# ColumbiaDVMM/ColumbiaImageSearch

Measured on AMD Instinct MI355X. Metric: queries/sec @ recall@10 on 10M LOPQ index, higher is better.
Workload: dtype f64

## Files before the change

### columbiaimagesearch_amd/csrc/lopq_scan3.hip

```cpp
#include "scan_common.h"
#include <cmath>
#include <cstdio>
#include <cstdlib>

typedef unsigned short u16x2_t __attribute__((ext_vector_type(2)));

static __device__ __forceinline__ uint32_t pk_add_u16(uint32_t a, uint32_t b) {
    return __builtin_bit_cast(uint32_t, (u16x2_t)(__builtin_bit_cast(u16x2_t, a) + __builtin_bit_cast(u16x2_t, b)));
}
static __device__ __forceinline__ uint32_t pk_subsat_u16(uint32_t a, uint32_t b) {
    return __builtin_bit_cast(uint32_t, __builtin_elementwise_sub_sat(__builtin_bit_cast(u16x2_t, a), __builtin_bit_cast(u16x2_t, b)));
}

static __device__ __forceinline__ uint32_t pk_min_u16(uint32_t a, uint32_t b) {
    return __builtin_bit_cast(uint32_t, __builtin_elementwise_min(__builtin_bit_cast(u16x2_t, a), __builtin_bit_cast(u16x2_t, b)));
}

static const int S3G = 4;

#ifdef CIS_S3_COUNTERS
__device__ unsigned long long g_s3_ctr[16];
#define S3_CLK() ((long long)__builtin_amdgcn_s_memtime())
#define S3_CTR(i, v) do { if (threadIdx.x == 0) atomicAdd(&g_s3_ctr[i], (unsigned long long)(v)); } while (0)
extern "C" int cis_debug_counters3(unsigned long long* out, int reset) {
// ... 60 lines not shown
        if (boundW < lds_ld(&sh->wt[w])) lds_st(&sh->wt[w], boundW);
    }
    __builtin_amdgcn_fence(__ATOMIC_RELEASE, "workgroup");
    uint32_t thr = bound_to_thr(block_bound<NW>(sh), qs.inv_up);
    uint32_t cut = thr;
    int W = cap - L;
    W = W > 24 ? 24 : (W < 0 ? 0 : W);
    if (wave_count_le<NR>(keep, s, cut) > L + W) {
        const uint32_t v = wave_bisect_window<NR>(keep, s, mn, mx, L, W);
        const uint32_t vm = v + (uint32_t)M;
        if (wave_count_le<NR>(keep, s, vm) > cap) return -1;
        const uint64_t boundL = val_to_bound(v, M, qs.ub);
        if (lane == 0) {
            if (boundL < lds_ld(&sh->wl[w])) lds_st(&sh->wl[w], boundL);
        }
        __builtin_amdgcn_fence(__ATOMIC_RELEASE, "workgroup");
        thr = bound_to_thr(block_bound<NW>(sh), qs.inv_up);
        cut = vm < thr ? vm : thr;
    }
    if (lane == 0) {
        if (thr < lds_ld(&sh->thr)) lds_st(&sh->thr, thr);
    }
    return wave_stable_keep<NR>([&](int r) { return keep[r] && s[r] <= cut; }, [&](int r, int idx) { rk[idx] = ent[r]; });
}

template <int M, int NR, int NW>
__device__ __forceinline__ int wave_compact3_exact(uint32_t* rk, int cnt, int L, int Lw, const QScale& qs, Scan3Shared* sh, int w,
                                                   const uint8_t* __restrict__ codes, int64_t start, int K,
                                                   const double* __restrict__ t0, const double* __restrict__ t1, uint32_t& dup_pos) {
    const int lane = threadIdx.x & 63;
    uint32_t hi[NR], lo[NR], ent[NR];
    bool keep[NR];
    uint32_t mn = 0xffffffffu, mx = 0u;
#pragma unroll
    for (int r = 0; r < NR; ++r) {
        const int e = r * 64 + lane;
        keep[r] = e < cnt;
        ent[r] = keep[r] ? rk[e] : 0xffffffffu;
        hi[r] = 0xffffffffu;
        lo[r] = 0xffffffffu;
    }
#pragma unroll
    for (int r = 0; r < NR; ++r) {
        if (r * 64 >= cnt) break;
        const CodeWords<M> cw = load_code<M>(codes, start + (keep[r] ? (ent[r] & 0xffffu) : 0u));
        const uint64_t k = keep[r] ? (uint64_t)__double_as_longlong(adc64_words<M>(cw.w, K, t0, t1)) : ~0ull;
        hi[r] = (uint32_t)(k >> 32);
        lo[r] = (uint32_t)k;
        mn = (keep[r] && hi[r] < mn) ? hi[r] : mn;
        mx = (keep[r] && hi[r] > mx) ? hi[r] : mx;
    }
    wave_minmax_all(mn, mx);
    uint32_t vhiL;
    uint64_t boundL;
    wave_exact_cut<NR>(hi, lo, keep, [&](int r) { return ent[r] & 0xffffu; }, mn, mx, cnt, L, vhiL, boundL, dup_pos);
    const uint64_t boundW = (cnt >= Lw) ? hi_to_bound(wave_kth_bisect<NR>(hi, keep, mn, vhiL, Lw)) : 0x7ff0000000000000ull;
    if (lane == 0) {
        if (boundW < lds_ld(&sh->wt[w])) lds_st(&sh->wt[w], boundW);
        if (boundL < lds_ld(&sh->wl[w])) lds_st(&sh->wl[w], boundL);
    }
    __builtin_amdgcn_fence(__ATOMIC_RELEASE, "workgroup");
    const uint64_t bound = block_bound<NW>(sh);
    if (lane == 0) {
        const uint32_t thr = bound_to_thr(bound, qs.inv_up);
        if (thr < lds_ld(&sh->thr)) lds_st(&sh->thr, thr);
    }
    return wave_stable_keep<NR>([&](int r) { return keep[r] && (((uint64_t)hi[r] << 32) | lo[r]) <= bound; },
                                [&](int r, int idx) { rk[idx] = ent[r]; });
}

template <int NR, int NW>
__device__ __forceinline__ int wave_filter3(uint32_t* rk, int cnt, const QScale& qs, const Scan3Shared* sh) {
    const int lane = threadIdx.x & 63;
    const uint32_t thr = bound_to_thr(block_bound<NW>(sh), qs.inv_up);
    uint32_t k[NR];
#pragma unroll
    for (int r = 0; r < NR; ++r) {
        const int e = r * 64 + lane;
        k[r] = e < cnt ? rk[e] : 0xffffffffu;
    }
    return wave_stable_keep<NR>([&](int r) { return (r * 64 + lane < cnt) && ((k[r] >> 16) <= thr); }, [&](int r, int idx) { rk[idx] = k[r]; });
}

template <int M, int OCT>
__device__ __forceinline__ void adc16_issue(const uint32_t (&D)[(M + 3) / 4], int o, const char* __restrict__ tab,
                                            const RotConsts<M>& rc, u32x2_t (&f)[OCT]) {
    constexpr int SH = ((M == 4) ? 2 : (M == 8 ? 3 : 4)) + 3;
#pragma unroll
    for (int i = 0; i < OCT; ++i) {
        const int t = o * OCT + i;
        const uint32_t k = __builtin_amdgcn_ubfe(D[t >> 2], rc.sh[t & 3], 8);
        f[i] = *reinterpret_cast<const u32x2_t*>(tab + ((k << SH) | (rc.cj[t] << 1)));
    }
}

template <int OCT>
__device__ __forceinline__ u32x2_t adc16_sum(const u32x2_t (&f)[OCT]) {
    uint32_t a0 = f[0][0], a1 = f[0][1];
#pragma unroll
    for (int i = 1; i < OCT; ++i) {
        a0 = pk_add_u16(a0, f[i][0]);
        a1 = pk_add_u16(a1, f[i][1]);
    }
    u32x2_t r;
    r[0] = a0; r[1] = a1;
    return r;
}

static __device__ __forceinline__ uint32_t ld16(const uint16_t* p) { return *reinterpret_cast<const volatile uint16_t*>(p); }
static __device__ __forceinline__ void st16(uint16_t* p, uint32_t v) { *reinterpret_cast<volatile uint16_t*>(p) = (uint16_t)v; }

template <int M, int NR, int U, int NW>
__device__ __forceinline__ void scan3_group(const WorkItem* __restrict__ items, const TabDesc* __restrict__ tabs,
                                            const int (&item_idx)[S3G], int ng,
                                            const double* __restrict__ T, const float* __restrict__ T32,
                                            const uint8_t* __restrict__ codes, int K, int L, int S,
                                            uint64_t* __restrict__ item_surv, int* __restrict__ item_n, float* __restrict__ item_slack,
                                            unsigned long long* __restrict__ qbound, char* smem, bool two_pass) {
    constexpr int G = S3G;
    constexpr int R = NR * 64 - 8;
    constexpr int nf = M / 2;
    constexpr int OCT = M >= 8 ? 8 : 4, NU = M / OCT;
    constexpr uint32_t CAP = 65535u / M;
    char* tab = smem;
    uint32_t* rk_all = reinterpret_cast<uint32_t*>(smem + (size_t)K * M * G * 2);
    Scan3Shared* sh = reinterpret_cast<Scan3Shared*>(rk_all + G * NW * R);
    uint16_t* thr1 = reinterpret_cast<uint16_t*>(sh + G);
    const int tid = threadIdx.x, lane = tid & 63;
    const int w = __builtin_amdgcn_readfirstlane(tid >> 6);
    const long long c0 = S3_CLK();
    (void)c0;
    const WorkItem it0 = items[item_idx[0]];
    {
        int tab0[G], tab1[G];
        float qinv[G];
#pragma unroll
        for (int g = 0; g < G; ++g) {
            tab0[g] = items[item_idx[g]].tab0; tab1[g] = items[item_idx[g]].tab1;
            float mxT = fmaxf(__int_as_float(tabs[tab0[g]].pad), __int_as_float(tabs[tab1[g]].pad));
            mxT = fmaxf(mxT, 1e-30f);
            float qi = ((float)CAP / mxT) * (1.0f - 9.5367431640625e-7f);
            qi = (mxT < 3.0e38f) ? qi : 0.0f;
            qi = (qi < 3.0e38f) ? qi : 3.0e38f;
            qinv[g] = qi;
        }
        if (tid < G) {
            const int g = tid;
            float qi = qinv[0];
#pragma unroll
            for (int gg = 1; gg < G; ++gg) qi = (g == gg) ? qinv[gg] : qi;
            const double inv_up = (double)qi * (1.0 + 2.384185791015625e-7);
            const double ub = qi > 0.0f ? (1.0 + 4.76837158203125e-7) / (double)qi : __longlong_as_double(0x7ff0000000000000LL);
            sh[g].inv_up = inv_up;
            sh[g].ub = ub;
            const unsigned long long e = (g < ng) ? __hip_atomic_load(&qbound[items[item_idx[g]].q], __ATOMIC_RELAXED, __HIP_MEMORY_SCOPE_AGENT)
                                                  : 0x7ff0000000000000ull;
            sh[g].ext = e;
            uint32_t thr = (g < ng) ? bound_to_thr(e, inv_up) : 0u;
#ifdef CIS_S3_PROBE_NOPASS
            thr = 0u;
            if (true) { sh[g].thr = 0u; thr1[g] = 0; } else
#endif
            { sh[g].thr = thr; thr1[g] = (uint16_t)((g < ng) ? thr + 1u : 0u); }
            if (g < ng) {
                item_slack[2 * (int64_t)item_idx[g] + 0] = __double2float_ru(ub * ((double)M + 0.1));
                item_slack[2 * (int64_t)item_idx[g] + 1] = __double2float_ru(ub);
            }
        }
        if (tid < 8 * G) {
            const int g = tid >> 3, i = tid & 7;
            sh[g].wt[i] = 0x7ff0000000000000ull; sh[g].wl[i] = 0x7ff0000000000000ull;
            sh[g].wcnt[i] = 0;
        }
        const int nvec = (nf * K) >> 2;
        uint32_t* tw = reinterpret_cast<uint32_t*>(tab);
// ... 460 lines not shown
    const uint8_t* __restrict__ codes, int K, int L, int S, int* __restrict__ queue_ctr ,
    uint64_t* __restrict__ item_surv, int* __restrict__ item_n, float* __restrict__ item_slack,
    unsigned long long* __restrict__ qbound , int two_pass, int single_queue ) {
    extern __shared__ __attribute__((aligned(16))) char smem[];
    constexpr int G = S3G;
    constexpr int R = NR * 64 - 8;
    int* s_next = reinterpret_cast<int*>(smem + (size_t)K * M * G * 2 + (size_t)G * NW * R * 4 + G * sizeof(Scan3Shared) + 32);
    const int* qs = n_slots_ptr + 8;
    const int home = blockIdx.x & 7;
    const long long k0 = S3_CLK();
    (void)k0;
    for (int a = 0; a < 8; ++a) {
        const int x = (home + a) & 7;
        const int qstart = qs[x];
        const int count = single_queue ? (x == 0 ? qs[1] - qstart : 0) : qs[x + 1] - qstart;
        if (count <= 0) continue;
        while (true) {
            const long long q0 = S3_CLK();
            (void)q0;
            int j;
            if constexpr (NW > 1) {
                __syncthreads();
                if (threadIdx.x == 0) *s_next = atomicAdd(&queue_ctr[x], 1);
                __syncthreads();
                j = __builtin_amdgcn_readfirstlane(*s_next);
            } else {
                int t = 0;
                if (threadIdx.x == 0) t = atomicAdd(&queue_ctr[x], 1);
                j = __builtin_amdgcn_readfirstlane(t);
            }
            S3_CTR(8, S3_CLK() - q0);
            if (j >= count) break;
            const int slot = qstart + j;
            int idx[G];
            int ng = 0;
            bool same = true;
#pragma unroll
            for (int g = 0; g < G; ++g) {
                idx[g] = slots[slot * G + g];
                if (idx[g] >= 0) {
                    ng = g + 1;
                    same = same && items[idx[g]].start == items[idx[0]].start && items[idx[g]].len == items[idx[0]].len;
                } else {
                    idx[g] = idx[0];
                }
            }
            if (!same) {
                for (int g2 = 0; g2 < ng; ++g2) {
                    int oi[G];
#pragma unroll
                    for (int g = 0; g < G; ++g) {
                        oi[g] = idx[0];
#pragma unroll
                        for (int gg = 1; gg < G; ++gg)
                            if (gg == g2) oi[g] = idx[gg];
                    }
                    if (g2 > 0) __syncthreads();
                    scan3_group<M, NR, U, NW>(items, tabs, oi, 1, T, T32, codes, K, L, S, item_surv, item_n, item_slack, qbound, smem, two_pass != 0);
                }
                continue;
            }
            scan3_group<M, NR, U, NW>(items, tabs, idx, ng, T, T32, codes, K, L, S, item_surv, item_n, item_slack, qbound, smem, two_pass != 0);
        }
    }
    S3_CTR(9, S3_CLK() - k0);
    S3_CTR(10, 1);
}

struct Slot4 {
    int item[S3G], tab0[S3G], tab1[S3G], q[S3G];
    float qinv[S3G];
    int start_lo, start_hi, len, ng;
    int ist_lo[S3G], ist_hi[S3G], ilen[S3G];
};
struct Scan4Shared {
    double inv_up, ub;
    uint64_t ext;
    uint32_t tau;
    int verify;
    int cnt;
    int q;
};

template <int M, int UU, int OCT = (M >= 8 ? 8 : 4)>
__device__ __forceinline__ void adc16_rows(const CodeWords<M> (&cur)[UU], const char* __restrict__ tab, const RotConsts<M>& rc,
                                           u32x2_t (&d)[UU]) {
    constexpr int NU = M / OCT;
    u32x2_t fbuf[2][OCT];
    uint32_t D[2][(M + 3) / 4];
    rot_words<M>(cur[0], rc, D[0]);
    adc16_issue<M, OCT>(D[0], 0, tab, rc, fbuf[0]);
#pragma unroll
    for (int q = 0; q < UU * NU; ++q) {
        const int u = q / NU, o = q % NU;
        if (q + 1 < UU * NU) {
            const int u1 = (q + 1) / NU, o1 = (q + 1) % NU;
            if (o1 == 0) rot_words<M>(cur[u1], rc, D[u1 & 1]);
            adc16_issue<M, OCT>(D[u1 & 1], o1, tab, rc, fbuf[(q + 1) & 1]);
        }
        __builtin_amdgcn_sched_barrier(0);
        const u32x2_t part = adc16_sum<OCT>(fbuf[q & 1]);
        if (o == 0) {
            d[u] = part;
        } else {
            d[u][0] = pk_add_u16(d[u][0], part[0]);
            d[u][1] = pk_add_u16(d[u][1], part[1]);
        }
        __builtin_amdgcn_sched_barrier(0);
    }
}

static __device__ __forceinline__ void lds_barrier() {
    asm volatile("s_waitcnt lgkmcnt(0)\n\ts_barrier" ::: "memory");
}

#ifndef CIS_S4_U
#define CIS_S4_U 2
#endif
#ifndef CIS_S4_UL
#define CIS_S4_UL 2
#endif
#ifndef CIS_S4_OCT
#define CIS_S4_OCT 4
#endif
#ifndef CIS_S4_WPE
#define CIS_S4_WPE 6
#endif
static const int S4_OCT = CIS_S4_OCT;
#ifndef CIS_S4_DEFER
#define CIS_S4_DEFER 1
#endif
#ifndef CIS_S4_NW_LONG
#define CIS_S4_NW_LONG 4
#endif
#ifndef CIS_S4_NW_SHORT
#define CIS_S4_NW_SHORT 4
#endif
#ifndef CIS_S4_WPE8
#define CIS_S4_WPE8 6
#endif
#ifndef CIS_S4_GLISTS
#define CIS_S4_GLISTS 0
#endif
#ifndef CIS_S4_WPE_LONG
#define CIS_S4_WPE_LONG 6
#endif
#ifndef CIS_S4_PF
#define CIS_S4_PF 2
#endif
#ifndef CIS_S4_LCAP
#define CIS_S4_LCAP 504
#endif
#ifndef CIS_S4_NS
#define CIS_S4_NS 16
#endif
#ifndef CIS_S4_Z
#define CIS_S4_Z 4.0f
#endif
static const int S4_DS = 8;
static const int S4_LCAP = CIS_S4_LCAP;
static const int S4_NS = CIS_S4_NS;

static const int S4_LCAP_LONG = 1016;

static size_t scan4_lds(int M, int K, int lcap, int nw) {
    const bool glists = lcap > 504 && CIS_S4_DEFER != 0 && CIS_S4_GLISTS != 0;
    const size_t lists = glists ? (size_t)nw * ((32 / nw) * 128) * 2 : (size_t)S3G * lcap * 4, samp = glists ? 0 : (size_t)S3G * S4_NS * 64 * 2;
    return (size_t)K * M * S3G * 2 + (lists > samp ? lists : samp) + S3G * sizeof(Scan4Shared) + 32 + (size_t)S3G * nw * 4 + (S4_DS + 1) * sizeof(Slot4);
}

static __device__ __forceinline__ int sample_row(int t, int nrows, int ns) { return (int)(((uint32_t)t * (uint32_t)nrows) / (uint32_t)ns); }

template <int M, int U, int NW, int WPE, int LCAPT>
__global__ __launch_bounds__(NW * 64) __attribute__((amdgpu_waves_per_eu(WPE, WPE))) void k_adc_scan4(
    const WorkItem* __restrict__ items, const TabDesc* __restrict__ tabs, const int* __restrict__ slots,
    const int* __restrict__ n_slots_ptr, const float* __restrict__ T32 , const double* __restrict__ T,
    const uint8_t* __restrict__ codes, int K, int L, int S,
    int* __restrict__ dbg , int* __restrict__ fhdr ,
    int* __restrict__ fslots, uint64_t* __restrict__ item_surv, int* __restrict__ item_n, float* __restrict__ item_slack,
    unsigned long long* __restrict__ qbound, float zq , int frac_den ,
    int nsx , int dyn ,
    float sat ) {
    extern __shared__ __attribute__((aligned(16))) char smem[];
    constexpr int G = S3G;
    static_assert(NW >= G && NW % G == 0 && NW <= 8, "waves 0 .. G-1 serve one query each in the threshold and verification phases");
    static_assert(M == 4 || M == 8 || M == 16, "float4s of the half tables are dealt to the threads in rounds of 256");
    constexpr int nf = M / 2;
    constexpr uint32_t CAP = 65535u / M;
    constexpr int LCAP = LCAPT, NS = S4_NS, NRV = (LCAP + 63) / 64;
    constexpr bool GLISTS = (LCAPT > 504) && (CIS_S4_DEFER != 0) && (CIS_S4_GLISTS != 0);
    constexpr size_t LIST_B_FULL = (size_t)G * LCAP * 4 > (size_t)G * NS * 64 * 2 ? (size_t)G * LCAP * 4 : (size_t)G * NS * 64 * 2;
    constexpr size_t LIST_B = GLISTS ? (size_t)NW * (((LCAPT > 504 ? 32 : 16) / NW) * 128) * 2 : LIST_B_FULL;
    char* tab = smem;
    uint32_t* lists = reinterpret_cast<uint32_t*>(smem + (size_t)K * M * G * 2);
    uint16_t* samp = reinterpret_cast<uint16_t*>(lists);
    Scan4Shared* sh = reinterpret_cast<Scan4Shared*>(reinterpret_cast<char*>(lists) + LIST_B);
    uint16_t* thr1 = reinterpret_cast<uint16_t*>(sh + G);
    int* s_flag = reinterpret_cast<int*>(thr1 + 4);
    int* s_cnt = s_flag + 1;
    int* wcnt = reinterpret_cast<int*>(reinterpret_cast<char*>(thr1) + 32);
    Slot4* sd = reinterpret_cast<Slot4*>(reinterpret_cast<char*>(thr1) + 32 + G * NW * 4);
#ifdef CIS_S4_SHARED_LISTS
    constexpr bool WLISTS = LCAPT > 504;
#else
    constexpr bool WLISTS = true;
#endif
    constexpr int WCAP = LCAPT / NW;
    constexpr int PCAP_LDS = (int)(LIST_B / (NW * 2));
    constexpr int NRP = (LCAPT > 504 ? 32 : 16) / NW;
    constexpr int PCAP = NRP * 128 < PCAP_LDS ? NRP * 128 : PCAP_LDS;
    static_assert(PCAP % 2 == 0 && (PCAP_LDS * 2) % 4 == 0, "position lists are read back as 32-bit pairs");
    const int tid = threadIdx.x, lane = tid & 63;
    const int w = __builtin_amdgcn_readfirstlane(tid >> 6);
    const int total = n_slots_ptr[0];
    const int xcd = blockIdx.x & 7, lb = blockIdx.x >> 3;
    const int LW = gridDim.x >> 3;
    auto slot_of = [&](int k) -> int {
        const int li = lb + k * LW;
        const int j = (((li >> 5) * 8 + xcd) << 5) | (li & 31);
        return j < total ? j : -1;
    };
    const RotConsts<M> rc = make_rot<M>(lane);
    const int nvec = (nf * K) >> 2;
    const long long k0 = S3_CLK();
    (void)k0;
    for (int kb = 0;; kb += S4_DS) {
        int dyn_j = -1;
        if (LCAPT > 504 && dyn) {
            __syncthreads();
            if (tid == 0) {
                int jn = -1;
                if (dyn == 1) {
                    jn = atomicAdd(&dbg[6], 1);
                    jn = jn < total ? jn : -1;
                } else {
                    int* qx = dbg - 9;
                    for (int a2 = 0; a2 < 8 && jn < 0; ++a2) {
                        const int x = (xcd + a2) & 7;
                        const int li = atomicAdd(&qx[x], 1);
                        const int jj = (((li >> 5) * 8 + x) << 5) | (li & 31);
                        if (jj < total) jn = jj;
                    }
                }
                *s_flag = jn;
            }
            __syncthreads();
            dyn_j = *s_flag;
            if (dyn_j < 0) break;
        } else {
            if (slot_of(kb) < 0) break;
        }
        __syncthreads();
        if (tid < S4_DS) {
            Slot4 d;
            int dyn_s = dyn;
            asm volatile("" : "+s"(dyn_s));
            const int j = (LCAPT > 504 && dyn_s) ? (tid == 0 ? dyn_j : -1) : slot_of(kb + tid);
            d.ng = 0; d.len = 0; d.start_lo = d.start_hi = 0;
#pragma unroll
            for (int g = 0; g < G; ++g) { d.item[g] = 0; d.tab0[g] = 0; d.tab1[g] = 0; d.q[g] = 0; d.qinv[g] = 0.f; d.ist_lo[g] = d.ist_hi[g] = d.ilen[g] = 0; }
            if (j >= 0) {
                int idx[G];
                int ng = 0;
                bool same = true;
#pragma unroll
                for (int g = 0; g < G; ++g) idx[g] = slots[j * G + g];
                const int64_t st0 = items[idx[0]].start;
                const int len0 = items[idx[0]].len;
#pragma unroll
                for (int g = 0; g < G; ++g) {
                    if (idx[g] >= 0) ng = g + 1;
                    else idx[g] = idx[0];
                    const WorkItem* it = &items[idx[g]];
                    same = same && it->start == st0 && it->len == len0;
                    const int t0 = it->tab0, t1 = it->tab1;
                    d.item[g] = idx[g]; d.tab0[g] = t0; d.tab1[g] = t1; d.q[g] = it->q;
                    d.ist_lo[g] = (int)(uint32_t)it->start; d.ist_hi[g] = (int)(it->start >> 32); d.ilen[g] = it->len;
                    float mxT = fmaxf(__int_as_float(tabs[t0].pad), __int_as_float(tabs[t1].pad));
                    mxT = fmaxf(mxT, 1e-30f);
                    float qi = ((float)CAP / mxT) * (1.0f - 9.5367431640625e-7f);
                    qi = (mxT < 3.0e38f) ? qi : 0.0f;
                    qi = (qi < 3.0e38f) ? qi : 3.0e38f;
                    d.qinv[g] = qi;
                }
                d.start_lo = (int)(uint32_t)st0; d.start_hi = (int)(st0 >> 32); d.len = len0;
                d.ng = same ? ng : -ng;
            }
            int tid_d = tid;
            asm volatile("" : "+v"(tid_d));
            sd[tid_d] = d;
        }
        __syncthreads();
        for (int kk = 0; kk < S4_DS; ++kk) {
            const Slot4* d = &sd[kk];
            const int ngs0 = __builtin_amdgcn_readfirstlane(d->ng);
            if (ngs0 == 0) break;
            int remaining = ngs0 < 0 ? ((1 << (-ngs0)) - 1) : 0;
            do {
            if (ngs0 < 0) {
                Slot4* ds = &sd[S4_DS];
                if (tid == 0) {
                    const Slot4* src = &sd[kk];
                    int g0 = 0;
                    while (!((remaining >> g0) & 1)) ++g0;
                    int n = 0, rest = remaining;
// ... 17 lines not shown
                remaining = __builtin_amdgcn_readfirstlane(ds->ist_lo[0]);
            }
            const int ngs = __builtin_amdgcn_readfirstlane(d->ng);
            const long long c0 = S3_CLK();
            (void)c0;
            const int ng = ngs;
            bool fail = false;
            if (!fail) {
                float qinv[G];
#pragma unroll
                for (int g = 0; g < G; ++g)
                    qinv[g] = __builtin_bit_cast(float, __builtin_amdgcn_readfirstlane(__builtin_bit_cast(int, d->qinv[g])));
                const int len = __builtin_amdgcn_readfirstlane(d->len);
                const int64_t start = ((int64_t)__builtin_amdgcn_readfirstlane(d->start_hi) << 32) | (uint32_t)__builtin_amdgcn_readfirstlane(d->start_lo);
                if (sat > 0.0f) {
                    if (w < G) {
                        const int g = w;
                        if (g < ng) {
                            const int t0 = __builtin_amdgcn_readfirstlane(d->tab0[g]), t1 = __builtin_amdgcn_readfirstlane(d->tab1[g]);
                            const int64_t Ta = (int64_t)t0 * nf * K, Tb = (int64_t)t1 * nf * K;
                            const int c = len >= 64 ? (int)(((int64_t)lane * len) >> 6) : lane;
                            uint32_t key = 0x7f7fffffu;
                            if (c < len) {
                                const CodeWords<M> cw = load_code<M>(codes, start + c);
                                float ds = 0.f;
#pragma unroll
                                for (int j = 0; j < M / 2; ++j) ds += tab_f1(T32, T, Ta + j * K + ((cw.w[j >> 2] >> (8 * (j & 3))) & 255u));
#pragma unroll
                                for (int j = 0; j < M / 2; ++j) ds += tab_f1(T32, T, Tb + j * K + ((cw.w[(M / 2 + j) >> 2] >> (8 * ((M / 2 + j) & 3))) & 255u));
                                key = __float_as_uint(fmaxf(ds, 0.f));
                            }
                            int rk = 4 + (int)((64 * (int64_t)L + len - 1) / len);
                            rk = rk > 48 ? 48 : rk;
                            uint32_t mn = key;
                            for (int r = 0; r < rk; ++r) {
                                uint32_t mx = 0u;
                                mn = key;
                                wave_minmax_step<1>(mn, mx); wave_minmax_step<2>(mn, mx); wave_minmax_step<4>(mn, mx);
                                wave_minmax_step<8>(mn, mx); wave_minmax_step<16>(mn, mx); wave_minmax_step<32>(mn, mx);
                                if (r + 1 < rk) {
                                    const uint64_t hit = __ballot(key == mn);
                                    if (lane == (int)__builtin_ctzll(hit)) key = 0x7f7fffffu;
                                }
                            }
                            const float d4 = __uint_as_float(mn);
                            const float qs = (sat * (float)CAP) / fmaxf(d4, 1e-30f);
                            const float q0 = d->qinv[g];
                            if (lane == 0 && q0 > 0.0f && qs > q0 && qs < 3.0e38f && d4 < 1.0e38f) const_cast<Slot4*>(d)->qinv[g] = qs;
                        }
                    }
                    lds_barrier();
#pragma unroll
                    for (int g = 0; g < G; ++g)
                        qinv[g] = __builtin_bit_cast(float, __builtin_amdgcn_readfirstlane(__builtin_bit_cast(int, d->qinv[g])));
                }
                int tid_st = tid;
                asm volatile("" : "+v"(tid_st));
                for (int vt = tid_st; vt < nvec; vt += NW * 64) {
                    const int j = vt & (nf - 1), kq = vt / nf, k0 = 4 * kq;
                    const int vidx = j * (K >> 2) + kq;
                    float4 pv[G][2];
#pragma unroll
                    for (int g = 0; g < G; ++g) {
                        const int t0 = __builtin_amdgcn_readfirstlane(d->tab0[g]), t1 = __builtin_amdgcn_readfirstlane(d->tab1[g]);
                        pv[g][0] = tab_f4(T32, T, t0, nf * K, vidx);
                        pv[g][1] = tab_f4(T32, T, t1, nf * K, vidx);
                    }
                    uint32_t* tw = reinterpret_cast<uint32_t*>(tab);
#pragma unroll
                    for (int s2 = 0; s2 < 2; ++s2) {
#pragma unroll
                        for (int c = 0; c < 4; ++c) {
                            uint32_t qv[G];
#pragma unroll
                            for (int g = 0; g < G; ++g) {
                                const float4 q = pv[g][s2];
                                const float x = c == 0 ? q.x : (c == 1 ? q.y : (c == 2 ? q.z : q.w));
                                qv[g] = (g < ng) ? (uint32_t)(x * qinv[g]) : CAP;
                                qv[g] = qv[g] > CAP ? CAP : qv[g];
                            }
                            u32x2_t pk;
                            pk[0] = qv[0] | (qv[1] << 16);
                            pk[1] = qv[2] | (qv[3] << 16);
                            *reinterpret_cast<u32x2_t*>(tw + (((k0 + c) * M + s2 * nf + j) << 1)) = pk;
                        }
                    }
                }
                if (tid >= 64 && tid < 64 + G) {
                    const int g = tid - 64;
                    float qi = qinv[0];
#pragma unroll
                    for (int gg = 1; gg < G; ++gg) qi = (g == gg) ? qinv[gg] : qi;
                    const double inv_up = (double)qi * (1.0 + 2.384185791015625e-7);
                    const double ub = qi > 0.0f ? (1.0 + 4.76837158203125e-7) / (double)qi : __longlong_as_double(0x7ff0000000000000LL);
                    const int item = d->item[g];
                    const int q = d->q[g];
                    sh[g].inv_up = inv_up;
                    sh[g].ub = ub;
                    sh[g].q = q;
                    sh[g].ext = (g < ng) ? __hip_atomic_load(&qbound[q], __ATOMIC_RELAXED, __HIP_MEMORY_SCOPE_AGENT) : 0x7ff0000000000000ull;
                    sh[g].cnt = 0;
                    s_cnt[g] = 0;
                    if (g < ng) {
                        item_slack[2 * (int64_t)item + 0] = __double2float_ru(ub * ((double)M + 0.1));
                        item_slack[2 * (int64_t)item + 1] = __double2float_ru(ub);
                    }
                }
                if (tid == 0) *s_flag = 0;
                __amdgpu_buffer_rsrc_t rs;
                {
                    const uint64_t cbase = (uint64_t)(uintptr_t)(codes + start * M);
                    const uint32_t blo = (uint32_t)__builtin_amdgcn_readfirstlane((int)(uint32_t)cbase);
                    const uint32_t bhi = (uint32_t)__builtin_amdgcn_readfirstlane((int)(uint32_t)(cbase >> 32));
                    rs = __builtin_amdgcn_make_buffer_rsrc((void*)(uintptr_t)(((uint64_t)bhi << 32) | blo), 0, len * M, 0x00020000);
                }
                const int nrows = (len + 63) >> 6;
                constexpr bool MULTI = LCAPT > 504;
                if constexpr (!MULTI) {
                    const int ns = nrows < NS ? nrows : NS;
                    constexpr int SPW = NS / NW;
                    static_assert(NS % (2 * NW) == 0, "sample rows come in pairs per wave");
                    CodeWords<M> sc[SPW];
                    int srow[SPW];
#pragma unroll
                    for (int i = 0; i < SPW; ++i) {
                        const int t = SPW * w + i;
                        srow[i] = t < ns ? sample_row(t, nrows, ns) : nrows;
                        sc[i] = load_code_buf<M>(rs, srow[i] * 64 + lane);
                    }
                    S3_CTR(11, S3_CLK() - c0);
                    lds_barrier();
                    S3_CTR(2, S3_CLK() - c0);
                    {
                        u32x2_t dd[SPW];
#if defined(CIS_S4_PROBE) && CIS_S4_PROBE >= 3
                        for (int u = 0; u < SPW; ++u) { dd[u][0] = 0xffffffffu; dd[u][1] = 0xffffffffu; }
#else
                        adc16_rows<M, SPW, S4_OCT>(sc, tab, rc, dd);
#endif
#pragma unroll
                        for (int u = 0; u < SPW; ++u) {
                            const int t = SPW * w + u;
                            const bool ok = (t < ns) && (srow[u] * 64 + lane < len);
#pragma unroll
                            for (int g = 0; g < G; ++g) {
                                const uint32_t sg = (g & 1) ? (dd[u][g >> 1] >> 16) : (dd[u][g >> 1] & 0xffffu);
#if defined(CIS_S4_PROBE) && CIS_S4_PROBE >= 3
                                samp[g * (NS * 64) + t * 64 + lane] = (uint16_t)0xffffu;
#else
                                samp[g * (NS * 64) + t * 64 + lane] = (uint16_t)(ok ? sg : 0xffffu);
#endif
                            }
                        }
                    }
                    lds_barrier();
                    S3_CTR(3, S3_CLK() - c0);
                    if (w < G) {
                        const int g = w;
                        uint32_t sv[NS];
                        int nsam = 0;
#pragma unroll
                        for (int r = 0; r < NS; ++r) {
                            sv[r] = samp[g * (NS * 64) + r * 64 + lane];
                            nsam += __popcll(__ballot(sv[r] != 0xffffu));
                        }
                        const bool exact = ns == nrows;
                        int ksv = L;
                        if (!exact) {
                            const float need = (float)L * (float)nsam / (float)len;
                            float zq_s = zq;
                            asm volatile("" : "+s"(zq_s));
                            const float hz = 0.5f * zq_s;
                            const float rt = hz + sqrtf(hz * hz + need);
                            ksv = (int)(rt * rt) + 1;
                        }
                        uint32_t tau = 65534u;
                        bool have_bound = false;
                        if (g < ng && nsam >= ksv) {
                            uint32_t lo = 0u, hi = 65534u;
                            while (lo < hi) {
                                const uint32_t p = lo + ((hi - lo) >> 1);
                                int c = 0;
#pragma unroll
                                for (int r = 0; r < NS; ++r) c += __popcll(__ballot(sv[r] <= p));
                                if (c >= ksv) hi = p;
                                else lo = p + 1;
                            }
                            tau = lo;
                            have_bound = tau < (sat > 0.f ? CAP - (uint32_t)M - 2u : 65534u);
                        }
                        if (lane == 0) {
                            uint32_t keep = 65534u;
                            if (have_bound) {
                                keep = tau + (uint32_t)M + 1u;
                                keep = keep < 65534u ? keep : 65534u;
                            }
                            const uint32_t t_ext = (g < ng) ? bound_to_thr(sh[g].ext, sh[g].inv_up) : 0u;
                            const uint32_t t = keep < t_ext ? keep : t_ext;
                            thr1[g] = (uint16_t)((g < ng) ? t + 1u : 0u);
#if defined(CIS_S4_PROBE) && CIS_S4_PROBE == 1
                            thr1[g] = 0;
#endif
                            sh[g].tau = tau;
                            sh[g].verify = (have_bound && keep < t_ext && !exact) ? 1 : 0;
#if defined(CIS_S4_PROBE)
                            sh[g].verify = 0;
#endif
                        }
                    }
                } else {
                    int ns = nrows / frac_den;
                    ns = ns < NS ? NS : ns;
                    ns = ns > nsx ? nsx : ns;
                    ns = ns < nrows ? ns : nrows;
                    constexpr int SPW = 4;
                    const int rounds = (ns + NW * SPW - 1) / (NW * SPW);
                    CodeWords<M> sc[SPW];
                    int srow[SPW];
#pragma unroll
                    for (int i = 0; i < SPW; ++i) {
                        const int t = SPW * w + i;
                        srow[i] = t < ns ? sample_row(t, nrows, ns) : nrows;
                        sc[i] = load_code_buf<M>(rs, srow[i] * 64 + lane);
                    }
                    S3_CTR(11, S3_CLK() - c0);
                    lds_barrier();
                    S3_CTR(2, S3_CLK() - c0);
                    {
                        uint32_t bm0 = 0xffffffffu, bm1 = 0xffffffffu;
#pragma unroll 1
                        for (int r = 0; r < rounds; ++r) {
                            CodeWords<M> nsc[SPW];
                            int nrow[SPW];
                            if constexpr (MULTI) {
                                if (r + 1 < rounds) {
#pragma unroll
                                    for (int i = 0; i < SPW; ++i) {
                                        const int t = ((r + 1) * NW + w) * SPW + i;
                                        nrow[i] = t < ns ? sample_row(t, nrows, ns) : nrows;
                                        nsc[i] = load_code_buf<M>(rs, nrow[i] * 64 + lane);
                                    }
                                }
                            }
                            u32x2_t dd[SPW];
#if defined(CIS_S4_PROBE) && CIS_S4_PROBE >= 3
                            for (int u = 0; u < SPW; ++u) { dd[u][0] = 0xffffffffu; dd[u][1] = 0xffffffffu; }
#else
                            adc16_rows<M, SPW, S4_OCT>(sc, tab, rc, dd);
#endif
#pragma unroll
                            for (int u = 0; u < SPW; ++u) {
                                const bool ok = srow[u] < nrows && (srow[u] * 64 + lane < len);
                                bm0 = pk_min_u16(bm0, ok ? dd[u][0] : 0xffffffffu);
                                bm1 = pk_min_u16(bm1, ok ? dd[u][1] : 0xffffffffu);
                            }
                            if constexpr (MULTI) {
                                if (r + 1 < rounds) {
#pragma unroll
                                    for (int i = 0; i < SPW; ++i) { sc[i] = nsc[i]; srow[i] = nrow[i]; }
                                }
                            }
                        }
                        u32x2_t bm;
                        bm[0] = bm0; bm[1] = bm1;
                        reinterpret_cast<u32x2_t*>(samp)[w * 64 + lane] = bm;
                    }
                    lds_barrier();
                    S3_CTR(3, S3_CLK() - c0);
                    if (w < G) {
                        const int g = w;
                        uint32_t sv[NW];
#pragma unroll
                        for (int r = 0; r < NW; ++r) {
                            const uint32_t xw = lds_ld(reinterpret_cast<const uint32_t*>(samp) + 2 * (r * 64 + lane) + (g >> 1));
                            sv[r] = (g & 1) ? (xw >> 16) : (xw & 0xffffu);
                        }
                        const bool all = ns == nrows;
                        const int nsam = all ? len : ns * 64;
                        int ksv = L;
                        if (!all) {
                            const float need = (float)L * (float)nsam / (float)len;
                            const float hz = 0.5f * zq;
                            const float rt = hz + sqrtf(hz * hz + need);
                            ksv = (int)(rt * rt) + 1;
                        }
                        uint32_t tau = 65534u;
                        bool have_bound = false;
                        if (g < ng && nsam >= ksv) {
                            uint32_t lo = 0u, hi = 65534u;
                            while (lo < hi) {
                                const uint32_t p = lo + ((hi - lo) >> 1);
                                int c = 0;
#pragma unroll
                                for (int r = 0; r < NW; ++r) c += __popcll(__ballot(sv[r] <= p));
                                if (c >= ksv) hi = p;
                                else lo = p + 1;
                            }
                            tau = lo;
                            have_bound = tau < (sat > 0.f ? CAP - (uint32_t)M - 2u : 65534u);
                        }
                        if (lane == 0) {
                            uint32_t keep = 65534u;
                            if (have_bound) {
                                keep = tau + (uint32_t)M + 1u;
                                keep = keep < 65534u ? keep : 65534u;
                            }
                            const uint32_t t_ext = (g < ng) ? bound_to_thr(sh[g].ext, sh[g].inv_up) : 0u;
                            const uint32_t t = keep < t_ext ? keep : t_ext;
                            thr1[g] = (uint16_t)((g < ng) ? t + 1u : 0u);
#if defined(CIS_S4_PROBE) && CIS_S4_PROBE == 1
                            thr1[g] = 0;
#endif
                            sh[g].tau = tau;
                            sh[g].verify = (have_bound && keep < t_ext && !all) ? 1 : 0;
#if defined(CIS_S4_PROBE)
                            sh[g].verify = 0;
#endif
                        }
                    }
                }
                lds_barrier();
                S3_CTR(4, S3_CLK() - c0);
                {
                    const uint64_t tp64 = lds_ld(reinterpret_cast<const uint64_t*>(thr1));
                    u32x2_t tpk;
                    tpk[0] = (uint32_t)tp64; tpk[1] = (uint32_t)(tp64 >> 32);
                    const uint32_t s01 = (uint32_t)__builtin_amdgcn_readfirstlane((int)tpk[0]);
                    const uint32_t s23 = (uint32_t)__builtin_amdgcn_readfirstlane((int)tpk[1]);
#if defined(CIS_S4_PROBE) && CIS_S4_PROBE >= 2
                    const int nit = 0;
#else
                    const int nit = (len + 64 * U - 1) / (64 * U);
#endif
                    constexpr int PF = CIS_S4_PF;
                    CodeWords<M> ring[PF][U];
#pragma unroll
                    for (int k = 0; k < PF; ++k) {
#pragma unroll
                        for (int u = 0; u < U; ++u) ring[k][u] = load_code_buf<M>(rs, (w + k * NW) * 64 * U + u * 64 + lane);
                        __builtin_amdgcn_sched_barrier(0);
                    }
                    int wcur[G];
#pragma unroll
                    for (int g = 0; g < G; ++g) wcur[g] = 0;
#if CIS_S4_DEFER
                    uint16_t* plist = reinterpret_cast<uint16_t*>(lists) + (size_t)w * PCAP_LDS;
                    int pcur = 0;
#endif
                    for (int iter0 = w; iter0 < nit; iter0 += NW * PF) {
#pragma unroll
                      for (int k = 0; k < PF; ++k) {
                        const int iter = iter0 + k * NW;
                        const int base = iter * 64 * U;
                        u32x2_t dd[U];
                        adc16_rows<M, U, S4_OCT>(ring[k], tab, rc, dd);
#pragma unroll
                        for (int u = 0; u < U; ++u) ring[k][u] = load_code_buf<M>(rs, (iter + PF * NW) * 64 * U + u * 64 + lane);
#pragma unroll
                        for (int u = 0; u < U; ++u) {
                            const uint32_t xx = pk_subsat_u16(tpk[0], dd[u][0]) | pk_subsat_u16(tpk[1], dd[u][1]);
                            unsigned long long am = __ballot(xx != 0u);
                            const int n = len - base - u * 64;
                            if (n < 64) am &= n <= 0 ? 0ull : ((1ull << n) - 1ull);
                            if (am == 0ull) continue;
#if CIS_S4_DEFER
                            if constexpr (WLISTS) {
                                const int idx = __builtin_amdgcn_mbcnt_hi((unsigned)(am >> 32), __builtin_amdgcn_mbcnt_lo((unsigned)am, pcur));
                                if (((am >> lane) & 1ull) && idx < PCAP) plist[idx] = (uint16_t)(base + u * 64 + lane);
                                pcur += __popcll(am);
                                continue;
                            }
#endif
                            if constexpr (WLISTS) {
#ifdef CIS_S4_SCALAR_APPEND
                                while (am != 0ull) {
                                    const int l = __builtin_ctzll(am);
                                    am &= am - 1ull;
                                    const uint32_t d0 = (uint32_t)__builtin_amdgcn_readlane((int)dd[u][0], l);
                                    const uint32_t d1 = (uint32_t)__builtin_amdgcn_readlane((int)dd[u][1], l);
                                    const uint32_t pos = (uint32_t)(base + u * 64 + l);
#pragma unroll
                                    for (int g = 0; g < G; ++g) {
                                        const uint32_t dw = (g >> 1) ? d1 : d0;
                                        const uint32_t sg = (g & 1) ? (dw >> 16) : (dw & 0xffffu);
                                        const uint32_t t1 = (g & 1) ? ((g >> 1) ? s23 >> 16 : s01 >> 16) : ((g >> 1) ? s23 & 0xffffu : s01 & 0xffffu);
                                        if (sg < t1) {
                                            if (wcur[g] < WCAP) lists[(g * NW + w) * WCAP + wcur[g]] = (sg << 16) | pos;
                                            wcur[g] += 1;
                                        }
                                    }
                                }
#else
#pragma unroll
                                for (int g = 0; g < G; ++g) {
                                    const uint32_t sg = (g & 1) ? (dd[u][g >> 1] >> 16) : (dd[u][g >> 1] & 0xffffu);
                                    const uint32_t t1 = (g & 1) ? ((g >> 1) ? s23 >> 16 : s01 >> 16) : ((g >> 1) ? s23 & 0xffffu : s01 & 0xffffu);
                                    const unsigned long long mg = __ballot(sg < t1) & am;
                                    if (mg == 0ull) continue;
                                    const int idx = __builtin_amdgcn_mbcnt_hi((unsigned)(mg >> 32), __builtin_amdgcn_mbcnt_lo((unsigned)mg, wcur[g]));
                                    if (((mg >> lane) & 1ull) && idx < WCAP) lists[(g * NW + w) * WCAP + idx] = (sg << 16) | (uint32_t)(base + u * 64 + lane);
                                    wcur[g] += __popcll(mg);
                                }
#endif
                                continue;
                            }
                            unsigned long long m[G];
                            int mine = 0;
#pragma unroll
                            for (int g = 0; g < G; ++g) {
                                const uint32_t sg = (g & 1) ? (dd[u][g >> 1] >> 16) : (dd[u][g >> 1] & 0xffffu);
                                const uint32_t t1 = (g & 1) ? ((g >> 1) ? s23 >> 16 : s01 >> 16) : ((g >> 1) ? s23 & 0xffffu : s01 & 0xffffu);
                                m[g] = __ballot(sg < t1) & am;
                                mine = (lane == g) ? __popcll(m[g]) : mine;
                            }
                            int got = 0;
                            if (lane < G) got = atomicAdd(&s_cnt[lane], mine);
#pragma unroll
                            for (int g = 0; g < G; ++g) {
                                if (m[g] == 0ull) continue;
                                const int b0 = __builtin_amdgcn_readlane(got, g);
                                const uint32_t sg = (g & 1) ? (dd[u][g >> 1] >> 16) : (dd[u][g >> 1] & 0xffffu);
                                const int idx = __builtin_amdgcn_mbcnt_hi((unsigned)(m[g] >> 32), __builtin_amdgcn_mbcnt_lo((unsigned)m[g], b0));
                                if (((m[g] >> lane) & 1ull) && idx < LCAP) lists[g * LCAP + idx] = (sg << 16) | (uint32_t)(base + u * 64 + lane);
                            }
                        }
                      }
                    }
                    S3_CTR(13, S3_CLK() - c0);
#if CIS_S4_DEFER
                    if constexpr (WLISTS) {
                        const bool pover = pcur > PCAP;
                        const int pn = pover ? 0 : pcur;
                        static_assert(NRP * 128 <= PCAP_LDS, "the NRP registers are read from the wave's own position list");
                        uint32_t pp[NRP];
#pragma unroll
                        for (int r = 0; r < NRP; ++r) pp[r] = lds_ld(reinterpret_cast<const uint32_t*>(plist) + r * 64 + lane);
                        auto on_of = [&](int it) -> bool { return 2 * (((it >> 1) * 64) + lane) + (it & 1) < pn; };
                        CodeWords<M> cw[2];
                        cw[0] = load_code_buf<M>(rs, on_of(0) ? (int)(pp[0] & 0xffffu) : len);
                        cw[1] = load_code_buf<M>(rs, on_of(1) ? (int)(pp[0] >> 16) : len);
                        lds_barrier();
                        uint32_t* grow[G];
#pragma unroll
                        for (int g = 0; g < G; ++g)
                            grow[g] = reinterpret_cast<uint32_t*>(item_surv + (int64_t)__builtin_amdgcn_readfirstlane(d->item[g]) * S);
                        if (pn > 0) {
                            const int nreg = (pn + 127) >> 7;
#pragma unroll 1
                            for (int r = 0; r < nreg; ++r) {
                              const uint32_t cur = pp[0];
#pragma unroll
                              for (int k = 0; k + 1 < NRP; ++k) pp[k] = pp[k + 1];
                              pp[NRP - 1] = 0u;
#pragma unroll
                              for (int h = 0; h < 2; ++h) {
                                const int it = 2 * r + h;
                                const uint32_t pos = h ? (cur >> 16) : (cur & 0xffffu);
                                CodeWords<M> cc[1];
                                cc[0] = cw[h];
                                u32x2_t d1[1];
                                adc16_rows<M, 1, S4_OCT>(cc, tab, rc, d1);
                                cw[h] = load_code_buf<M>(rs, on_of(it + 2) ? (int)(h ? (pp[0] >> 16) : (pp[0] & 0xffffu)) : len);
                                const unsigned long long am2 = __ballot(on_of(it));
#pragma unroll
                                for (int g = 0; g < G; ++g) {
                                    const uint32_t sg = (g & 1) ? (d1[0][g >> 1] >> 16) : (d1[0][g >> 1] & 0xffffu);
                                    const uint32_t t1 = (g & 1) ? ((g >> 1) ? s23 >> 16 : s01 >> 16) : ((g >> 1) ? s23 & 0xffffu : s01 & 0xffffu);
                                    const unsigned long long mg = __ballot(sg < t1) & am2;
                                    if (mg == 0ull) continue;
                                    const int idx = __builtin_amdgcn_mbcnt_hi((unsigned)(mg >> 32), __builtin_amdgcn_mbcnt_lo((unsigned)mg, wcur[g]));
                                    if (((mg >> lane) & 1ull) && idx < WCAP) {
                                        if constexpr (GLISTS) grow[g][w * WCAP + idx] = (sg << 16) | pos;
                                        else lists[(g * NW + w) * WCAP + idx] = (sg << 16) | pos;
                                    }
                                    wcur[g] += __popcll(mg);
                                }
                              }
                            }
                        }
                        if (pover) wcur[0] = WCAP + 1;
                    }
#endif
                    if constexpr (WLISTS) {
                        if (lane < G) {
                            int c = wcur[0];
#pragma unroll
                            for (int g = 1; g < G; ++g) c = (lane == g) ? wcur[g] : c;
                            wcnt[lane * NW + w] = c;
                        }
                    }
                }
                S3_CTR(12, S3_CLK() - c0);
                if constexpr (GLISTS) __syncthreads();
                else lds_barrier();
                S3_CTR(5, S3_CLK() - c0);
                bool bad = false;
                if (w < ng) {
                    const int g = w;
                    int tot = 0;
                    int wtot[NW];
                    int lane_v = lane;
                    asm volatile("" : "+v"(lane_v));
                    if constexpr (WLISTS) {
#pragma unroll
                        for (int r = 0; r < NW; ++r) {
                            wtot[r] = wcnt[g * NW + r];
                            bad = bad || wtot[r] > WCAP;
                            tot += wtot[r];
                        }
                    } else {
                        tot = s_cnt[g];
                        bad = tot > LCAP;
                    }
                    if (bad && lane_v == 0) atomicAdd(&dbg[2], 1);
                    if (!bad) {
                        uint32_t ent[NRV];
                        bool val[NRV];
#pragma unroll
                        for (int r = 0; r < NRV; ++r) {
                            if constexpr (WLISTS) {
                                constexpr int RW = NRV / NW;
                                const int e = (r % RW) * 64 + lane_v;
                                val[r] = e < wtot[r / RW];
                                if constexpr (GLISTS) {
                                    const uint32_t* gr = reinterpret_cast<const uint32_t*>(item_surv + (int64_t)__builtin_amdgcn_readfirstlane(d->item[g]) * S);
                                    ent[r] = val[r] ? __hip_atomic_load(gr + (r / RW) * WCAP + e, __ATOMIC_RELAXED, __HIP_MEMORY_SCOPE_AGENT) : 0xffffffffu;
                                } else {
                                    ent[r] = val[r] ? lists[(g * NW + r / RW) * WCAP + e] : 0xffffffffu;
                                }
                            } else {
                                val[r] = r * 64 + lane_v < tot;
                                ent[r] = val[r] ? lists[g * LCAP + r * 64 + lane_v] : 0xffffffffu;
                            }
                        }
                        const uint32_t tau = sh[g].tau;
                        if (sh[g].verify) {
                            int nle = 0;
#pragma unroll
                            for (int r = 0; r < NRV; ++r) nle += __popcll(__ballot(val[r] && (ent[r] >> 16) <= tau));
                            bad = nle < L;
                            if (bad && lane_v == 0) atomicAdd(&dbg[3], 1);
                        }
                        if (!bad) {
                            uint32_t cut = 65535u;
                            if (tot >= L) {
                                uint32_t mn = 0xffffffffu, mx = 0u;
#pragma unroll
                                for (int r = 0; r < NRV; ++r) {
                                    const uint32_t s = ent[r] >> 16;
                                    mn = (val[r] && s < mn) ? s : mn;
                                    mx = (val[r] && s > mx) ? s : mx;
                                }
                                wave_minmax_all(mn, mx);
                                uint32_t lo = mn, hi = mx;
                                while (lo < hi) {
                                    const uint32_t p = lo + ((hi - lo) >> 1);
                                    int c = 0;
#pragma unroll
                                    for (int r = 0; r < NRV; ++r) c += __popcll(__ballot(val[r] && (ent[r] >> 16) <= p));
                                    if (c >= L) {
                                        hi = p;
                                        if (c <= L + 16) break;
                                    } else {
                                        lo = p + 1;
                                    }
                                }
                                cut = hi + (uint32_t)M + 1u;
                                if (sat > 0.f && cut >= CAP) {
                                    bad = true;
                                    if (lane_v == 0) atomicAdd(&dbg[4], 1);
                                }
                                const uint64_t b = val_to_bound(hi, M, sh[g].ub);
                                if (lane_v == 0 && !bad && b < sh[g].ext) atomicMin(&qbound[sh[g].q], (unsigned long long)b);
                            } else if (sat > 0.f) {
                                bool sat = false;
#pragma unroll
                                for (int r = 0; r < NRV; ++r) sat = sat || (__ballot(val[r] && (ent[r] >> 16) + (uint32_t)M + 1u >= CAP) != 0ull);
                                if (sat) {
                                    bad = true;
                                    if (lane_v == 0) atomicAdd(&dbg[4], 1);
                                }
                            }
                            const int item = __builtin_amdgcn_readfirstlane(d->item[g]);
                            uint64_t* out = item_surv + (int64_t)item * S;
                            if constexpr (LCAP > 504) {
                                int nk = 0;
#pragma unroll
                                for (int r = 0; r < NRV; ++r) nk += __popcll(__ballot(val[r] && (ent[r] >> 16) <= cut));
                                if (nk > S) {
                                    bad = true;
                                    if (lane_v == 0) atomicAdd(&dbg[4], 1);
                                }
                            }
                            if (!bad) {
                                int kept = 0;
#pragma unroll
                                for (int r = 0; r < NRV; ++r) {
                                    const bool kp = val[r] && (ent[r] >> 16) <= cut;
                                    const unsigned long long mk = __ballot(kp);
                                    const int idx = kept + __builtin_amdgcn_mbcnt_hi((unsigned)(mk >> 32), __builtin_amdgcn_mbcnt_lo((unsigned)mk, 0));
                                    if (kp) out[idx] = ((uint64_t)(ent[r] >> 16) << 32) | (ent[r] & 0xffffu);
                                    kept += __popcll(mk);
                                }
                                if (lane_v == 0) item_n[item] = kept;
                            }
                        }
                    }
                    if (bad && lane_v == 0) *s_flag = 1;
                }
                lds_barrier();
                S3_CTR(6, S3_CLK() - c0);
// ... 543 lines not shown
```

Before: 24.11 million.

## Duplicate M=8 lookup tables in LDS to split bank traffic across two copies

For M=8 with long lists and non-global lists, the ADC half-tables are stored twice, interleaved in LDS. Lanes pick a copy by lane bit 3, which is meant to spread LDS bank accesses and cut conflicts in the table gathers. The survivor lists are packed into the unused slots of the interleaved table region so LDS footprint still allows four workgroups per CU. The deferred path also gets a simpler ballot-based survivor compaction. The cost is a doubled table write during setup, extra address arithmetic, and more intricate LDS aliasing.

```diff
diff --git a/columbiaimagesearch_amd/csrc/lopq_scan3.hip b/columbiaimagesearch_amd/csrc/lopq_scan3.hip
--- a/columbiaimagesearch_amd/csrc/lopq_scan3.hip
+++ b/columbiaimagesearch_amd/csrc/lopq_scan3.hip
@@ -166,15 +166,16 @@
     return wave_stable_keep<NR>([&](int r) { return (r * 64 + lane < cnt) && ((k[r] >> 16) <= thr); }, [&](int r, int idx) { rk[idx] = k[r]; });
 }
 
-template <int M, int OCT>
+template <int M, int OCT, bool TWO = false>
 __device__ __forceinline__ void adc16_issue(const uint32_t (&D)[(M + 3) / 4], int o, const char* __restrict__ tab,
                                             const RotConsts<M>& rc, u32x2_t (&f)[OCT]) {
-    constexpr int SH = ((M == 4) ? 2 : (M == 8 ? 3 : 4)) + 3;
+    constexpr int SH = ((M == 4) ? 2 : (M == 8 ? 3 : 4)) + 3 + (TWO ? 1 : 0);
 #pragma unroll
     for (int i = 0; i < OCT; ++i) {
         const int t = o * OCT + i;
         const uint32_t k = __builtin_amdgcn_ubfe(D[t >> 2], rc.sh[t & 3], 8);
-        f[i] = *reinterpret_cast<const u32x2_t*>(tab + ((k << SH) | (rc.cj[t] << 1)));
+        if constexpr (TWO) f[i] = *reinterpret_cast<const u32x2_t*>(tab + ((k << SH) + (rc.cj[t] << 1)));
+        else f[i] = *reinterpret_cast<const u32x2_t*>(tab + ((k << SH) | (rc.cj[t] << 1)));
     }
 }
 
@@ -801,21 +802,21 @@
     int q;
 };
 
-template <int M, int UU, int OCT = (M >= 8 ? 8 : 4)>
+template <int M, int UU, int OCT = (M >= 8 ? 8 : 4), bool TWO = false>
 __device__ __forceinline__ void adc16_rows(const CodeWords<M> (&cur)[UU], const char* __restrict__ tab, const RotConsts<M>& rc,
                                            u32x2_t (&d)[UU]) {
     constexpr int NU = M / OCT;
     u32x2_t fbuf[2][OCT];
     uint32_t D[2][(M + 3) / 4];
     rot_words<M>(cur[0], rc, D[0]);
-    adc16_issue<M, OCT>(D[0], 0, tab, rc, fbuf[0]);
+    adc16_issue<M, OCT, TWO>(D[0], 0, tab, rc, fbuf[0]);
 #pragma unroll
     for (int q = 0; q < UU * NU; ++q) {
         const int u = q / NU, o = q % NU;
         if (q + 1 < UU * NU) {
             const int u1 = (q + 1) / NU, o1 = (q + 1) % NU;
             if (o1 == 0) rot_words<M>(cur[u1], rc, D[u1 & 1]);
-            adc16_issue<M, OCT>(D[u1 & 1], o1, tab, rc, fbuf[(q + 1) & 1]);
+            adc16_issue<M, OCT, TWO>(D[u1 & 1], o1, tab, rc, fbuf[(q + 1) & 1]);
         }
         __builtin_amdgcn_sched_barrier(0);
         const u32x2_t part = adc16_sum<OCT>(fbuf[q & 1]);
@@ -882,7 +883,26 @@
 
 static const int S4_LCAP_LONG = 1016;
 
+static const int S4_TWO_NRP = 24;
+static constexpr bool scan4_two(int M, int lcap) { return M == 8 && lcap > 504 && CIS_S4_DEFER != 0 && CIS_S4_GLISTS == 0; }
+static constexpr size_t scan4_two_tab(int K, int lcap) {
+    const size_t t = (size_t)K * 8 * S3G * 4, l = (((size_t)S3G * lcap + 1) / 2) * 16;
+    return t > l ? t : l;
+}
+static constexpr size_t scan4_two_lds(int K, int lcap, int nw) {
+    return scan4_two_tab(K, lcap) + (size_t)S4_TWO_NRP * 128 * 2 + S3G * sizeof(Scan4Shared) + 32 + (size_t)S3G * nw * 4 + (S4_DS + 1) * sizeof(Slot4);
+}
+static_assert(4 * scan4_two_lds(256, S4_LCAP_LONG, 4) <= 163840, "the two-copy form keeps four workgroups of four waves per CU");
+static __device__ __forceinline__ RotConsts<8> two_copy_rot(const RotConsts<8>& rc, uint32_t copy) {
+    RotConsts<8> r2 = rc;
+#pragma unroll
+    for (int t = 0; t < 8; ++t) r2.cj[t] = (rc.cj[t] << 1) | (copy << 2);
+    return r2;
+}
+static __device__ __forceinline__ int two_list_byte(int i) { return ((i >> 1) << 4) + ((i & 1) << 2) + 8; }
+
 static size_t scan4_lds(int M, int K, int lcap, int nw) {
+    if (scan4_two(M, lcap)) return scan4_two_lds(K, lcap, nw);
     const bool glists = lcap > 504 && CIS_S4_DEFER != 0 && CIS_S4_GLISTS != 0;
     const size_t lists = glists ? (size_t)nw * ((32 / nw) * 128) * 2 : (size_t)S3G * lcap * 4, samp = glists ? 0 : (size_t)S3G * S4_NS * 64 * 2;
     return (size_t)K * M * S3G * 2 + (lists > samp ? lists : samp) + S3G * sizeof(Scan4Shared) + 32 + (size_t)S3G * nw * 4 + (S4_DS + 1) * sizeof(Slot4);
@@ -909,9 +929,11 @@
     constexpr int LCAP = LCAPT, NS = S4_NS, NRV = (LCAP + 63) / 64;
     constexpr bool GLISTS = (LCAPT > 504) && (CIS_S4_DEFER != 0) && (CIS_S4_GLISTS != 0);
     constexpr size_t LIST_B_FULL = (size_t)G * LCAP * 4 > (size_t)G * NS * 64 * 2 ? (size_t)G * LCAP * 4 : (size_t)G * NS * 64 * 2;
-    constexpr size_t LIST_B = GLISTS ? (size_t)NW * (((LCAPT > 504 ? 32 : 16) / NW) * 128) * 2 : LIST_B_FULL;
+    constexpr bool TWO = scan4_two(M, LCAPT);
+    constexpr size_t LIST_B = TWO ? (size_t)S4_TWO_NRP * 128 * 2 : (GLISTS ? (size_t)NW * (((LCAPT > 504 ? 32 : 16) / NW) * 128) * 2 : LIST_B_FULL);
+    static_assert(!TWO || LIST_B >= (size_t)NW * 64 * 8, "the bucket minima of the sample fit the position lists' region");
     char* tab = smem;
-    uint32_t* lists = reinterpret_cast<uint32_t*>(smem + (size_t)K * M * G * 2);
+    uint32_t* lists = reinterpret_cast<uint32_t*>(smem + (TWO ? scan4_two_tab(K, LCAPT) : (size_t)K * M * G * 2));
     uint16_t* samp = reinterpret_cast<uint16_t*>(lists);
     Scan4Shared* sh = reinterpret_cast<Scan4Shared*>(reinterpret_cast<char*>(lists) + LIST_B);
     uint16_t* thr1 = reinterpret_cast<uint16_t*>(sh + G);
@@ -926,7 +948,7 @@
 #endif
     constexpr int WCAP = LCAPT / NW;
     constexpr int PCAP_LDS = (int)(LIST_B / (NW * 2));
-    constexpr int NRP = (LCAPT > 504 ? 32 : 16) / NW;
+    constexpr int NRP = (TWO ? S4_TWO_NRP : (LCAPT > 504 ? 32 : 16)) / NW;
     constexpr int PCAP = NRP * 128 < PCAP_LDS ? NRP * 128 : PCAP_LDS;
     static_assert(PCAP % 2 == 0 && (PCAP_LDS * 2) % 4 == 0, "position lists are read back as 32-bit pairs");
     const int tid = threadIdx.x, lane = tid & 63;
@@ -939,7 +961,9 @@
         const int j = (((li >> 5) * 8 + xcd) << 5) | (li & 31);
         return j < total ? j : -1;
     };
-    const RotConsts<M> rc = make_rot<M>(lane);
+    RotConsts<M> rc = make_rot<M>(lane);
+    if constexpr (TWO) rc = two_copy_rot(rc, ((uint32_t)lane >> 3) & 1u);
+    auto list_at = [&](int i) -> uint32_t* { return reinterpret_cast<uint32_t*>(tab + two_list_byte(i)); };
     const int nvec = (nf * K) >> 2;
     const long long k0 = S3_CLK();
     (void)k0;
@@ -1123,7 +1147,13 @@
                             u32x2_t pk;
                             pk[0] = qv[0] | (qv[1] << 16);
                             pk[1] = qv[2] | (qv[3] << 16);
-                            *reinterpret_cast<u32x2_t*>(tw + (((k0 + c) * M + s2 * nf + j) << 1)) = pk;
+                            if constexpr (TWO) {
+                                u32x4_t pk2;
+                                pk2[0] = pk[0]; pk2[1] = pk[1]; pk2[2] = pk[0]; pk2[3] = pk[1];
+                                *reinterpret_cast<u32x4_t*>(tw + (((k0 + c) * M + s2 * nf + j) << 2)) = pk2;
+                            } else {
+                                *reinterpret_cast<u32x2_t*>(tw + (((k0 + c) * M + s2 * nf + j) << 1)) = pk;
+                            }
                         }
                     }
                 }
@@ -1287,7 +1317,7 @@
 #if defined(CIS_S4_PROBE) && CIS_S4_PROBE >= 3
                             for (int u = 0; u < SPW; ++u) { dd[u][0] = 0xffffffffu; dd[u][1] = 0xffffffffu; }
 #else
-                            adc16_rows<M, SPW, S4_OCT>(sc, tab, rc, dd);
+                            adc16_rows<M, SPW, S4_OCT, TWO>(sc, tab, rc, dd);
 #endif
 #pragma unroll
                             for (int u = 0; u < SPW; ++u) {
@@ -1394,14 +1424,25 @@
                         const int iter = iter0 + k * NW;
                         const int base = iter * 64 * U;
                         u32x2_t dd[U];
-                        adc16_rows<M, U, S4_OCT>(ring[k], tab, rc, dd);
+                        adc16_rows<M, U, S4_OCT, TWO>(ring[k], tab, rc, dd);
 #pragma unroll
                         for (int u = 0; u < U; ++u) ring[k][u] = load_code_buf<M>(rs, (iter + PF * NW) * 64 * U + u * 64 + lane);
 #pragma unroll
                         for (int u = 0; u < U; ++u) {
                             const uint32_t xx = pk_subsat_u16(tpk[0], dd[u][0]) | pk_subsat_u16(tpk[1], dd[u][1]);
+                            const int n = len - base - u * 64;
+#if CIS_S4_DEFER
+                            if constexpr (TWO) {
+                                const bool pass = xx != 0u && lane < n;
+                                const unsigned long long am = __builtin_amdgcn_ballot_w64(xx != 0u) & __builtin_amdgcn_ballot_w64(lane < n);
+                                if (am == 0ull) continue;
+                                const int idx = __builtin_amdgcn_mbcnt_hi((unsigned)(am >> 32), __builtin_amdgcn_mbcnt_lo((unsigned)am, pcur));
+                                if (pass && idx < PCAP) plist[idx] = (uint16_t)(base + u * 64 + lane);
+                                pcur += __popcll(am);
+                                continue;
+                            }
+#endif
                             unsigned long long am = __ballot(xx != 0u);
-                            const int n = len - base - u * 64;
                             if (n < 64) am &= n <= 0 ? 0ull : ((1ull << n) - 1ull);
                             if (am == 0ull) continue;
 #if CIS_S4_DEFER
@@ -1481,6 +1522,14 @@
                         cw[0] = load_code_buf<M>(rs, on_of(0) ? (int)(pp[0] & 0xffffu) : len);
                         cw[1] = load_code_buf<M>(rs, on_of(1) ? (int)(pp[0] >> 16) : len);
                         lds_barrier();
+                        RotConsts<M> rc0;
+                        if constexpr (TWO) {
+                            rc0 = rc;
+                            uint32_t keep0 = ~4u;
+                            asm volatile("" : "+v"(keep0));
+#pragma unroll
+                            for (int t = 0; t < M; ++t) rc0.cj[t] = rc.cj[t] & keep0;
+                        }
                         uint32_t* grow[G];
 #pragma unroll
                         for (int g = 0; g < G; ++g)
@@ -1500,7 +1549,8 @@
                                 CodeWords<M> cc[1];
                                 cc[0] = cw[h];
                                 u32x2_t d1[1];
-                                adc16_rows<M, 1, S4_OCT>(cc, tab, rc, d1);
+                                if constexpr (TWO) adc16_rows<M, 1, S4_OCT, true>(cc, tab, rc0, d1);
+                                else adc16_rows<M, 1, S4_OCT>(cc, tab, rc, d1);
                                 cw[h] = load_code_buf<M>(rs, on_of(it + 2) ? (int)(h ? (pp[0] >> 16) : (pp[0] & 0xffffu)) : len);
                                 const unsigned long long am2 = __ballot(on_of(it));
 #pragma unroll
@@ -1512,6 +1562,7 @@
                                     const int idx = __builtin_amdgcn_mbcnt_hi((unsigned)(mg >> 32), __builtin_amdgcn_mbcnt_lo((unsigned)mg, wcur[g]));
                                     if (((mg >> lane) & 1ull) && idx < WCAP) {
                                         if constexpr (GLISTS) grow[g][w * WCAP + idx] = (sg << 16) | pos;
+                                        else if constexpr (TWO) *list_at((g * NW + w) * WCAP + idx) = (sg << 16) | pos;
                                         else lists[(g * NW + w) * WCAP + idx] = (sg << 16) | pos;
                                     }
                                     wcur[g] += __popcll(mg);
@@ -1567,7 +1618,8 @@
                                     const uint32_t* gr = reinterpret_cast<const uint32_t*>(item_surv + (int64_t)__builtin_amdgcn_readfirstlane(d->item[g]) * S);
                                     ent[r] = val[r] ? __hip_atomic_load(gr + (r / RW) * WCAP + e, __ATOMIC_RELAXED, __HIP_MEMORY_SCOPE_AGENT) : 0xffffffffu;
                                 } else {
-                                    ent[r] = val[r] ? lists[(g * NW + r / RW) * WCAP + e] : 0xffffffffu;
+                                    if constexpr (TWO) ent[r] = val[r] ? *list_at((g * NW + r / RW) * WCAP + e) : 0xffffffffu;
+                                    else ent[r] = val[r] ? lists[(g * NW + r / RW) * WCAP + e] : 0xffffffffu;
                                 }
                             } else {
                                 val[r] = r * 64 + lane_v < tot;
```

After: 25.07 million, median of 6. 4.0% higher.
